# bd4sur/Nano

Hardware: AMD Instinct MI355X
Metric: decode_tokens_per_sec (higher is better)
Workload: dtype i8

## Files before the change

nano_amd/csrc/attn_impl.h:

```cpp
#pragma once
#include <hip/hip_fp16.h>
#include "device_common.h"
#include "kernels.h"

namespace nano {

namespace {

#ifndef NANO_GEMV_COMMON_H
#define DPP_F(v, ctrl) __int_as_float(__builtin_amdgcn_update_dpp(0, __float_as_int(v), (ctrl), 0xF, 0xF, true))
#endif

template <int W> __device__ __forceinline__ float group_sum_t(float v) {
    if (W >= 2) v += DPP_F(v, 0xB1);
    if (W >= 4) v += DPP_F(v, 0x4E);
    if (W >= 8) v += DPP_F(v, 0x141);
    if (W >= 16) v += DPP_F(v, 0x140);
    if (W >= 32) v += __shfl_xor(v, 16, 64);
    if (W >= 64) v += __shfl_xor(v, 32, 64);
    return v;
}
__device__ __forceinline__ float wave_sum_dpp(float v) {
    v += DPP_F(v, 0xB1); v += DPP_F(v, 0x4E); v += DPP_F(v, 0x141); v += DPP_F(v, 0x140);
    const float r0 = __int_as_float(__builtin_amdgcn_readlane(__float_as_int(v), 0));
// ... 46 lines not shown
    if constexpr (!KVH) row_base[elem] = v; else reinterpret_cast<__half *>(row_base)[elem] = __float2half_rn(v);
}
template <bool KVH> __device__ __forceinline__ KVRaw<KVH> kv_load4(__amdgpu_buffer_rsrc_t r, uint32_t off) {
    KVRaw<KVH> o;
    if constexpr (!KVH) o.v = bload_f4(r, off);
    else { typedef int i32x2 __attribute__((ext_vector_type(2))); const i32x2 t = __builtin_amdgcn_raw_buffer_load_b64(r, (int)off, 0, 0); o.v = make_uint2((uint32_t)t.x, (uint32_t)t.y); }
    return o;
}

typedef unsigned int u32x2_t __attribute__((ext_vector_type(2)));
__device__ __forceinline__ float xlane8(float v) { return __int_as_float(__builtin_amdgcn_update_dpp(0, __float_as_int(v), 0x128, 0xF, 0xF, true)); }
template <int LPR> __device__ __forceinline__ float xsub_sum(float v) {
    if (LPR <= 8) v += xlane8(v);
    { const u32x2_t r = __builtin_amdgcn_permlane16_swap(__float_as_uint(v), __float_as_uint(v), false, false); v = __uint_as_float(r[0]) + __uint_as_float(r[1]); }
    { const u32x2_t r = __builtin_amdgcn_permlane32_swap(__float_as_uint(v), __float_as_uint(v), false, false); v = __uint_as_float(r[0]) + __uint_as_float(r[1]); }
    return v;
}
template <int LPR> __device__ __forceinline__ float xsub_max(float v) {
    if (LPR <= 8) v = fmaxf(v, xlane8(v));
    { const u32x2_t r = __builtin_amdgcn_permlane16_swap(__float_as_uint(v), __float_as_uint(v), false, false); v = fmaxf(__uint_as_float(r[0]), __uint_as_float(r[1])); }
    { const u32x2_t r = __builtin_amdgcn_permlane32_swap(__float_as_uint(v), __float_as_uint(v), false, false); v = fmaxf(__uint_as_float(r[0]), __uint_as_float(r[1])); }
    return v;
}

__device__ __forceinline__ void combine_weights_lds(const float *mlh, uint32_t nsplit, float *wsh) {
    if (threadIdx.x < 64u) {
        const uint32_t s = threadIdx.x;
        const bool in = s < nsplit;
        const float mm = in ? mlh[2 * s] : -INFINITY;
        float v = in ? mlh[2 * s + 1] : 0.0f;
        float M = v > 0.0f ? mm : -INFINITY;
#pragma unroll
        for (int o = 32; o > 0; o >>= 1) M = fmaxf(M, __shfl_xor(M, o, 64));
        const float e = v > 0.0f ? expf(mm - M) : 0.0f;
        v = v * e;
        v += DPP_F(v, 0xB1); v += DPP_F(v, 0x4E); v += DPP_F(v, 0x141);
        float L = __int_as_float(__builtin_amdgcn_readlane(__float_as_int(v), 0));
        if (nsplit > 8u) {
            L += __int_as_float(__builtin_amdgcn_readlane(__float_as_int(v), 8));
            L += __int_as_float(__builtin_amdgcn_readlane(__float_as_int(v), 16));
            L += __int_as_float(__builtin_amdgcn_readlane(__float_as_int(v), 24));
        }
        if (nsplit > 32u) {
            L += __int_as_float(__builtin_amdgcn_readlane(__float_as_int(v), 32));
            L += __int_as_float(__builtin_amdgcn_readlane(__float_as_int(v), 40));
            L += __int_as_float(__builtin_amdgcn_readlane(__float_as_int(v), 48));
            L += __int_as_float(__builtin_amdgcn_readlane(__float_as_int(v), 56));
        }
        wsh[s] = e / L;
    }
    __syncthreads();
}
__device__ __forceinline__ uint32_t combine_slots(uint32_t nsplit) { return nsplit <= 8u ? 8u : nsplit <= 32u ? 32u : 64u; }

constexpr int NP = 2;

template <int LPR, int QV, int KVM, int MODE, bool KVH, bool PG, int NPT, bool W16, bool FUSE>
__device__ __forceinline__ void attention_body(const AttnArgs &a, unsigned char *smem, const uint32_t grp, const uint32_t b, const uint32_t split,
                                               const SlabHand &hh, const uint32_t hand_tag = 0u, const uint32_t hand_wait16 = 0u) {
    static_assert(!W16 || (KVH && QV % 4 == 0), "16-byte FP16 loads: two float4 slots per load");
    static_assert(!FUSE || (((MODE == 1 && LPR * QV * 4 == 128) || MODE == 2) && KVM == 1 && !KVH && !PG && LPR * QV * 4 <= 128),
                  "the fused launch: Qwen3 decode at head_dim 128, or the plain decode mode (no q/k norm, adjacent-pair RoPE: Nano) at head_dim <= 128; FP32 contiguous cache");
    constexpr int R = 256 / LPR;
    const int tid = threadIdx.x, lane = tid & 63;
    const int wid = __builtin_amdgcn_readfirstlane(tid >> 6);
    const uint32_t nsplit = a.nsplit;
    const uint32_t hd = (MODE == 1) ? (uint32_t)(QV * LPR * 4) : a.hd, half = hd >> 1, hd4 = (hd + 3) & ~3u;
    uint32_t kv_mul, g, h0;
    bool first_of_group;
    if constexpr (MODE != 0) {
        kv_mul = 1u << a.kvmul_log2;
        g = grp & ((1u << a.kv_log2) - 1u);
        const uint32_t sub_wg = grp >> a.kv_log2;
        h0 = (g << a.kvmul_log2) + sub_wg * KVM;
        first_of_group = sub_wg == 0;
    } else {
        kv_mul = a.n_head / a.n_kv_head;
        const bool xcd = a.kv_log2 != 0xffffffffu;
        g = xcd ? (grp & ((1u << a.kv_log2) - 1u)) : (grp * KVM) / kv_mul;
        h0 = xcd ? g * kv_mul + (grp >> a.kv_log2) * KVM : grp * KVM;
        first_of_group = (h0 % kv_mul) == 0;
    }
    constexpr bool G = MODE == 0;
    constexpr int VR = (KVM + 1 + 3) / 4;
    constexpr int JJ = (LPR == 16) ? 2 : 1;
    const bool fresh_k = G ? a.kraw != nullptr : true;
    const bool has_norm = G ? a.q_norm != nullptr : MODE == 1;
    const bool rq3 = G ? a.rope_qwen3 != 0 : MODE == 1;
    const bool has_rope = G ? a.rope_cos != nullptr : true;
    const uint32_t fixed_range = G ? a.fixed_range : 0u;
    const bool causal = G ? a.is_causal != 0 : true;
    float *const q_out = G ? a.q_out : nullptr;

    float *qh = reinterpret_cast<float *>(smem);
    float *kh = qh + KVM * hd4;
    float *redm = kh + hd4;
    float *redl = redm + KVM * 4;
    float *part = redl + KVM * 4;

    NANO_STAMP(a.stamps, 0, tid);
    if constexpr (MODE != 0)
        asm volatile("" :: "s"(a.q), "s"(a.kraw), "s"(a.kcache), "s"(a.vcache), "s"(a.pos), "s"(a.q_norm), "s"(a.k_norm), "s"(a.rope_cur),
                     "s"(a.out), "s"(a.ml), "s"(a.xba_out), "s"(a.nsplit), "s"(a.range_hint), "s"(a.layer), "s"(a.S), "s"(a.q_dim), "s"(a.kv_dim),
                     "s"(a.cache_bstride_rows), "s"(a.kv_log2), "s"(a.kvmul_log2), "s"(a.vraw), "s"(a.xf_out), "s"(a.pt_rows), "s"(a.kvrow));
    const uint32_t pos_ld = (MODE == 0 && a.fixed_range) ? 0u : a.pos[b];
    constexpr bool paged = PG;
    uint32_t prow_ld = 0u;
    if constexpr (PG) prow_ld = a.kvrow[b];
    constexpr uint32_t ESZ = KVH ? 2u : 4u;
    const size_t slot_rows = paged ? (size_t)a.layer * a.pool_rows : (size_t)b * a.cache_bstride_rows + (size_t)a.layer * a.S;
    const float *kc = reinterpret_cast<const float *>(reinterpret_cast<const unsigned char *>(a.kcache) + (slot_rows * a.kv_dim + (size_t)g * hd) * ESZ);
    const float *vc = reinterpret_cast<const float *>(reinterpret_cast<const unsigned char *>(a.vcache) + (slot_rows * a.kv_dim + (size_t)g * hd) * ESZ);
    const uint32_t cache_bytes = (paged ? a.pool_rows : fixed_range ? fixed_range : a.S) * a.kv_dim * ESZ;
    const __amdgpu_buffer_rsrc_t rk = mkrsrc(kc, cache_bytes - g * hd * ESZ);
    const __amdgpu_buffer_rsrc_t rv = mkrsrc(vc, cache_bytes - g * hd * ESZ);
    const uint32_t sub = (uint32_t)tid / LPR, j = (uint32_t)tid % LPR;
    auto fidx = [&](int q) -> uint32_t { return W16 ? 2u * (j + (uint32_t)LPR * (uint32_t)(q >> 1)) + (uint32_t)(q & 1) : j + (uint32_t)LPR * (uint32_t)q; };
    const uint32_t range_hint = fixed_range ? fixed_range : a.range_hint;

    constexpr bool REGQK = MODE != 0;
    constexpr bool SHARE = REGQK && !FUSE && KVM > 1;
    float4 qv[KVM][QV], kfresh[QV], vfresh[QV];
    float4 sv[SHARE ? QV : 1], snw[SHARE ? QV : 1];
    float4 qnw[QV], knw[QV], rcs[QV], rsn[QV];
    const __amdgpu_buffer_rsrc_t rq = mkrsrc(a.q + (size_t)b * a.q_dim, a.q_dim * 4u);
    const __amdgpu_buffer_rsrc_t rkr = mkrsrc(fresh_k ? a.kraw + (size_t)b * a.kv_dim : nullptr, fresh_k ? a.kv_dim * 4u : 0u);
    const bool fresh_v = KVH && a.vraw != nullptr;
    const __amdgpu_buffer_rsrc_t rvr = mkrsrc(fresh_v ? a.vraw + (size_t)b * a.kv_dim : nullptr, fresh_v ? a.kv_dim * 4u : 0u);
    const __amdgpu_buffer_rsrc_t rqn = mkrsrc(a.q_norm, has_norm ? hd * 4u : 0u);
    const __amdgpu_buffer_rsrc_t rkn = mkrsrc(a.k_norm, has_norm ? hd * 4u : 0u);
    float e0[VR][JJ], e1[VR][JJ], nw0[VR][JJ], nw1[VR][JJ];
    float rc[JJ], rs[JJ];
    const bool rope_staged = G ? (a.rope_cur != nullptr && fresh_k) : true;
    if constexpr (SHARE) {
        if (wid == 0) {
            const __amdgpu_buffer_rsrc_t rr = mkrsrc(a.rope_cur + (size_t)b * 2 * half, 2 * half * 4u);
            const bool isq = sub < (uint32_t)KVM, isk = sub == (uint32_t)KVM;
#pragma unroll
            for (int q = 0; q < QV; q++) {
                const uint32_t f = fidx(q);
                const uint32_t fo = (f * 4u < hd) ? f * 16u : OOB;
                const float4 xq = bload_f4(rq, (isq && fo != OOB) ? (h0 + sub) * hd * 4u + fo : OOB), xk = bload_f4(rkr, (isk && fo != OOB) ? g * hd * 4u + fo : OOB);
                sv[q] = isq ? xq : xk;
                if (MODE == 1) {
                    const float4 nq = bload_f4(rqn, isq ? fo : OOB), nk = bload_f4(rkn, isk ? fo : OOB);
                    snw[q] = isq ? nq : nk;
                    const uint32_t fr = f & (uint32_t)(QV * LPR / 2 - 1);
                    rcs[q] = bload_f4(rr, fo == OOB ? OOB : fr * 16u);
                    rsn[q] = bload_f4(rr, fo == OOB ? OOB : (half + fr * 4u) * 4u);
                } else {
                    const float c0 = bload_f(rr, fo == OOB ? OOB : (2u * f) * 4u), c1 = bload_f(rr, fo == OOB ? OOB : (2u * f + 1u) * 4u);
                    const float s0 = bload_f(rr, fo == OOB ? OOB : (half + 2u * f) * 4u), s1 = bload_f(rr, fo == OOB ? OOB : (half + 2u * f + 1u) * 4u);
                    rcs[q] = make_float4(c0, c1, 0.f, 0.f); rsn[q] = make_float4(s0, s1, 0.f, 0.f);
                }
            }
        }
        if constexpr (KVH) {
#pragma unroll
            for (int q = 0; q < QV; q++) { const uint32_t f = fidx(q); vfresh[q] = bload_f4(rvr, (f * 4u < hd) ? g * hd * 4u + f * 16u : OOB); }
        }
    } else if constexpr (REGQK) {
        const __amdgpu_buffer_rsrc_t rr = mkrsrc(a.rope_cur + (size_t)b * 2 * half, 2 * half * 4u);
#pragma unroll
        for (int q = 0; q < QV; q++) {
            const uint32_t f = fidx(q);
            const uint32_t fo = (f * 4u < hd) ? f * 16u : OOB;
// ... 28 lines not shown
            const uint32_t qb = (h0 + v) * hd * 4u, kb = g * hd * 4u;
            e0[vr][jj] = isq ? bload_f(rq, o0 + (ok ? qb : 0u)) : isk ? bload_f(rkr, o0 + (ok ? kb : 0u)) : 0.0f;
            e1[vr][jj] = isq ? bload_f(rq, o1 + (ok ? qb : 0u)) : isk ? bload_f(rkr, o1 + (ok ? kb : 0u)) : 0.0f;
            nw0[vr][jj] = !has_norm ? 1.0f : isq ? bload_f(rqn, o0) : isk ? bload_f(rkn, o0) : 0.0f;
            nw1[vr][jj] = !has_norm ? 1.0f : isq ? bload_f(rqn, o1) : isk ? bload_f(rkn, o1) : 0.0f;
        }
    }
    {
        const __amdgpu_buffer_rsrc_t rr = mkrsrc(rope_staged ? a.rope_cur + (size_t)b * 2 * half : nullptr, rope_staged ? 2 * half * 4u : 0u);
#pragma unroll
        for (int jj = 0; jj < JJ; jj++) {
            const uint32_t pi = (uint32_t)lane + 64u * jj;
            rc[jj] = bload_f(rr, pi < half ? pi * 4u : OOB);
            rs[jj] = bload_f(rr, pi < half ? (half + pi) * 4u : OOB);
        }
    }
    }
    KVRaw<KVH> kreg[NPT][QV], vreg[NPT][QV];
    auto issue_kv = [&](uint32_t round) {
#pragma unroll
        for (int p = 0; p < NPT; p++) {
            const uint32_t tb = ((round * NPT + p) * nsplit + split) * R, t = tb + sub;
            uint32_t row = t;
            if constexpr (PG) {
                const uint32_t blk = tb >> 6;
                uint32_t rb = 0xffffffffu;
                if (blk < a.pt_stride && tb < range_hint) {
                    const uint64_t pa = reinterpret_cast<uint64_t>(a.pt_rows + (size_t)b * a.pt_bstride + blk);
                    const uint64_t pu = ((uint64_t)(uint32_t)__builtin_amdgcn_readfirstlane((uint32_t)(pa >> 32)) << 32) | (uint64_t)(uint32_t)__builtin_amdgcn_readfirstlane((uint32_t)pa);
                    asm volatile("s_nop 4\n\ts_load_dword %0, %1, 0x0\n\ts_waitcnt lgkmcnt(0)" : "=s"(rb) : "s"(pu) : "memory");
                }
                row = rb == 0xffffffffu ? 0x7fffffu : rb + (t & 63u);
            }
#pragma unroll
            for (int q = 0; q < QV; q++) {
                const uint32_t f = fidx(q);
                const uint32_t off = (f * 4u < hd && t < range_hint && row < 0x7fffffu) ? (row * a.kv_dim + f * 4u) * ESZ : OOB;
                if constexpr (W16) {
                    if ((q & 1) == 0) {
                        const i32x4 kk = __builtin_amdgcn_raw_buffer_load_b128(rk, (int)off, 0, 0), vv = __builtin_amdgcn_raw_buffer_load_b128(rv, (int)off, 0, 0);
                        kreg[p][q].v = make_uint2((uint32_t)kk.x, (uint32_t)kk.y); kreg[p][q + 1].v = make_uint2((uint32_t)kk.z, (uint32_t)kk.w);
                        vreg[p][q].v = make_uint2((uint32_t)vv.x, (uint32_t)vv.y); vreg[p][q + 1].v = make_uint2((uint32_t)vv.z, (uint32_t)vv.w);
                    }
                } else {
                    kreg[p][q] = kv_load4<KVH>(rk, off);
                    vreg[p][q] = kv_load4<KVH>(rv, off);
                }
            }
        }
    };
    issue_kv(0);
    __builtin_amdgcn_sched_barrier(0);
    NANO_STAMP(a.stamps, 1, tid);
    if constexpr (FUSE) {
        float *vh = part + 4 * KVM * hd4;
        const uint32_t t7 = (uint32_t)tid & 127u;
        const unsigned long long *hand = hh.buf;
        const unsigned long long *g0p = (uint32_t)tid < 128u ? hand + (size_t)h0 * hd + t7 : hand + hh.base[1] + (size_t)g * hd + t7;
        const unsigned long long *g1p = hand + hh.base[2] + (size_t)g * hd + t7;
        const unsigned long long tag_done = (unsigned long long)hand_tag << 32;
        unsigned long long g0 = 0, g1 = 0;
        const bool live7 = MODE == 1 || t7 < hd;
        const bool two = (uint32_t)tid < 128u && live7;
        auto sweep = [&](unsigned long long &x0, unsigned long long &x1) {
            x0 = live7 ? __hip_atomic_load(g0p, __ATOMIC_RELAXED, __HIP_MEMORY_SCOPE_AGENT) : tag_done;
            x1 = two ? __hip_atomic_load(g1p, __ATOMIC_RELAXED, __HIP_MEMORY_SCOPE_AGENT) : tag_done;
        };
        auto ready = [&](unsigned long long x0, unsigned long long x1) { return __all((uint32_t)(x0 >> 32) == hand_tag && (uint32_t)(x1 >> 32) == hand_tag) != 0; };
        unsigned long long a0, a1, b0, b1;
        for (uint32_t w_ = 0; w_ < hand_wait16; w_++) __builtin_amdgcn_s_sleep(16);
        sweep(a0, a1);
        bool got = false;
        for (uint32_t spin = 0; spin < (1u << 13); spin++) {
            sweep(b0, b1);
            if (ready(a0, a1)) { g0 = a0; g1 = a1; got = true; break; }
            sweep(a0, a1);
            if (ready(b0, b1)) { g0 = b0; g1 = b1; got = true; break; }
            if ((spin & 63u) == 63u && hand_aborted(hh)) break;
        }
        if (live7) {
            if ((uint32_t)tid < 128u) { qh[t7] = __uint_as_float((uint32_t)g0); vh[t7] = __uint_as_float((uint32_t)g1); }
            else kh[t7] = __uint_as_float((uint32_t)g0);
        }
        if (__syncthreads_or(got ? 0 : 1)) {
            if (!got && lane == 0) hand_give_up(hh, a.err);
            return;
        }
#pragma unroll
        for (int q = 0; q < QV; q++) {
            const uint32_t f = fidx(q);
            const bool in = MODE == 1 || f * 4u < hd;
            const float4 z4 = make_float4(0.f, 0.f, 0.f, 0.f);
            qv[0][q] = in ? *reinterpret_cast<const float4 *>(qh + 4u * f) : z4;
            kfresh[q] = in ? *reinterpret_cast<const float4 *>(kh + 4u * f) : z4;
            vfresh[q] = in ? *reinterpret_cast<const float4 *>(vh + 4u * f) : z4;
        }
    }

    const uint32_t pos = fixed_range ? (fixed_range - 1) : pos_ld;
    const uint32_t prow = paged ? prow_ld : pos;
    const uint32_t range = fixed_range ? fixed_range : (causal ? (pos + 1) : a.S);
    if constexpr (SHARE) {
        if (wid == 0) {
            const bool isq = sub < (uint32_t)KVM, isk = sub == (uint32_t)KVM;
            if (MODE == 1) {
                float ssq = 0.0f;
#pragma unroll
                for (int q = 0; q < QV; q++) { ssq += sv[q].x * sv[q].x; ssq += sv[q].y * sv[q].y; ssq += sv[q].z * sv[q].z; ssq += sv[q].w * sv[q].w; }
                ssq = group_sum_t<LPR>(ssq); ssq /= (float)hd; ssq += 1e-5f; ssq = 1.0f / sqrtf(ssq);
#pragma unroll
                for (int q = 0; q < QV; q++) {
                    sv[q].x = snw[q].x * (ssq * sv[q].x); sv[q].y = snw[q].y * (ssq * sv[q].y); sv[q].z = snw[q].z * (ssq * sv[q].z); sv[q].w = snw[q].w * (ssq * sv[q].w);
                }
#pragma unroll
                for (int q = 0; q < QV / 2; q++) {
                    const float4 l = sv[q], h = sv[q + QV / 2], c = rcs[q], sn = rsn[q];
                    sv[q].x = l.x * c.x - h.x * sn.x; sv[q + QV / 2].x = h.x * c.x + l.x * sn.x;
                    sv[q].y = l.y * c.y - h.y * sn.y; sv[q + QV / 2].y = h.y * c.y + l.y * sn.y;
                    sv[q].z = l.z * c.z - h.z * sn.z; sv[q + QV / 2].z = h.z * c.z + l.z * sn.z;
                    sv[q].w = l.w * c.w - h.w * sn.w; sv[q + QV / 2].w = h.w * c.w + l.w * sn.w;
                }
            } else {
#pragma unroll
                for (int q = 0; q < QV; q++) {
                    const float4 t = sv[q], c = rcs[q], sn = rsn[q];
                    sv[q].x = t.x * c.x - t.y * sn.x; sv[q].y = t.x * sn.x + t.y * c.x;
                    sv[q].z = t.z * c.y - t.w * sn.y; sv[q].w = t.z * sn.y + t.w * c.y;
                }
            }
            if (isk) {
#pragma unroll
                for (int q = 0; q < QV; q++) sv[q] = kv_round<KVH>(sv[q]);
            }
            if (isq || isk) {
                float *dst = isq ? qh + sub * hd4 : kh;
#pragma unroll
                for (int q = 0; q < QV; q++) { const uint32_t f = fidx(q); if (f * 4u < hd) *reinterpret_cast<float4 *>(dst + 4u * f) = sv[q]; }
            }
            if (isk && split == 0 && first_of_group) {
                float *krow = reinterpret_cast<float *>(reinterpret_cast<unsigned char *>(const_cast<float *>(kc)) + (size_t)prow * a.kv_dim * ESZ);
                float *vrow = reinterpret_cast<float *>(reinterpret_cast<unsigned char *>(const_cast<float *>(vc)) + (size_t)prow * a.kv_dim * ESZ);
#pragma unroll
                for (int q = 0; q < QV; q++) {
                    const uint32_t f = fidx(q);
                    if (f * 4u < hd) { kv_store4<KVH>(krow, 4u * f, sv[q]); if (KVH && fresh_v) kv_store4<KVH>(vrow, 4u * f, kv_round<KVH>(vfresh[q])); }
                }
            }
        }
        if (a.prep_only) return;
        __syncthreads();
#pragma unroll
        for (int q = 0; q < QV; q++) {
            const uint32_t f = fidx(q);
            const bool ok = f * 4u < hd;
#pragma unroll
            for (int m = 0; m < KVM; m++) qv[m][q] = ok ? *reinterpret_cast<const float4 *>(qh + m * hd4 + 4 * f) : make_float4(0.f, 0.f, 0.f, 0.f);
            kfresh[q] = ok ? *reinterpret_cast<const float4 *>(kh + 4 * f) : make_float4(0.f, 0.f, 0.f, 0.f);
            if (KVH) vfresh[q] = kv_round<KVH>(vfresh[q]);
        }
    } else if constexpr (REGQK) {
        if (MODE == 1) {
            float sk = 0.0f, sq[KVM];
#pragma unroll
            for (int m = 0; m < KVM; m++) sq[m] = 0.0f;
#pragma unroll
            for (int q = 0; q < QV; q++) {
                sk += kfresh[q].x * kfresh[q].x; sk += kfresh[q].y * kfresh[q].y; sk += kfresh[q].z * kfresh[q].z; sk += kfresh[q].w * kfresh[q].w;
// ... 57 lines not shown
            const uint32_t pi = (uint32_t)lane + 64u * jj;
            const bool ok = has_rope && pi < half && fresh_k;
            rc[jj] = ok ? a.rope_cos[(size_t)pos * half + pi] : 1.0f;
            rs[jj] = ok ? a.rope_sin[(size_t)pos * half + pi] : 0.0f;
        }
    }
#pragma unroll
    for (int vr = 0; vr < VR; vr++) {
        const uint32_t v = (uint32_t)wid + 4u * vr;
        if (v <= (uint32_t)KVM) {
            const bool isk = v == (uint32_t)KVM;
            float x0[JJ], x1[JJ];
#pragma unroll
            for (int jj = 0; jj < JJ; jj++) { x0[jj] = e0[vr][jj]; x1[jj] = e1[vr][jj]; }
            if (fresh_k && has_norm) {
                float acc = 0.0f;
#pragma unroll
                for (int jj = 0; jj < JJ; jj++) { acc += x0[jj] * x0[jj]; acc += x1[jj] * x1[jj]; }
                float ss = wave_sum_dpp(acc);
                ss /= (float)hd; ss += 1e-5f; ss = 1.0f / sqrtf(ss);
#pragma unroll
                for (int jj = 0; jj < JJ; jj++) { x0[jj] = nw0[vr][jj] * (ss * x0[jj]); x1[jj] = nw1[vr][jj] * (ss * x1[jj]); }
            }
            float *dst = isk ? kh : qh + v * hd4;
#pragma unroll
            for (int jj = 0; jj < JJ; jj++) {
                const uint32_t pi = (uint32_t)lane + 64u * jj;
                if (pi < half && (!isk || fresh_k)) {
                    const uint32_t i0 = rq3 ? pi : 2 * pi, i1 = rq3 ? pi + half : 2 * pi + 1;
                    float y0 = x0[jj], y1 = x1[jj];
                    if (fresh_k && has_rope) {
                        const float c = rc[jj], s = rs[jj];
                        if (rq3) { y0 = x0[jj] * c - x1[jj] * s; y1 = x1[jj] * c + x0[jj] * s; }
                        else { y0 = x0[jj] * c - x1[jj] * s; y1 = x0[jj] * s + x1[jj] * c; }
                    }
                    if (isk) { y0 = kv_round1<KVH>(y0); y1 = kv_round1<KVH>(y1); }
                    dst[i0] = y0; dst[i1] = y1;
                    if (isk && split == 0 && first_of_group) {
                        float *krow = reinterpret_cast<float *>(reinterpret_cast<unsigned char *>(const_cast<float *>(kc)) + (size_t)prow * a.kv_dim * ESZ);
                        kv_store1<KVH>(krow, i0, y0); kv_store1<KVH>(krow, i1, y1);
                    }
                    if (!isk && split == 0 && q_out) { float *qo = q_out + (size_t)b * a.q_dim + (size_t)(h0 + v) * hd; qo[i0] = y0; qo[i1] = y1; }
                }
            }
        }
    }
    if constexpr (KVH) {
#pragma unroll
        for (int q = 0; q < QV; q++) {
            const uint32_t f = fidx(q);
            const bool ok = f * 4u < hd;
            vfresh[q] = kv_round<KVH>(bload_f4(rvr, ok ? g * hd * 4u + f * 16u : OOB));
            if (fresh_v && ok && split == 0 && sub == 0 && first_of_group)
                kv_store4<KVH>(reinterpret_cast<float *>(reinterpret_cast<unsigned char *>(const_cast<float *>(vc)) + (size_t)prow * a.kv_dim * ESZ), 4u * f, vfresh[q]);
        }
    }
    __syncthreads();
    if (a.prep_only) return;

#pragma unroll
    for (int q = 0; q < QV; q++) {
        const uint32_t f = fidx(q);
        const bool ok = f * 4u < hd;
#pragma unroll
        for (int m = 0; m < KVM; m++) qv[m][q] = ok ? *reinterpret_cast<const float4 *>(qh + m * hd4 + 4 * f) : make_float4(0.f, 0.f, 0.f, 0.f);
        kfresh[q] = (ok && fresh_k) ? *reinterpret_cast<const float4 *>(kh + 4 * f) : make_float4(0.f, 0.f, 0.f, 0.f);
    }
    }
    NANO_STAMP(a.stamps, 2, qv[0][0].x);
    const float sq_hd = sqrtf((float)hd);
    float mrun[KVM], lrun[KVM];
    float4 acc[KVM][QV];
#pragma unroll
    for (int m = 0; m < KVM; m++) {
        mrun[m] = -INFINITY; lrun[m] = 0.0f;
#pragma unroll
        for (int q = 0; q < QV; q++) acc[m][q] = make_float4(0.f, 0.f, 0.f, 0.f);
    }
    const uint32_t per_round = NPT * nsplit * R;
    const uint32_t limit = range < range_hint ? range : range_hint;
    const uint32_t nround = (limit + per_round - 1) / per_round;
    for (uint32_t round = 0; round < nround; round++) {
        if (round) issue_kv(round);
        float sc[KVM][NPT];
#pragma unroll
        for (int p = 0; p < NPT; p++) {
            const uint32_t t = ((round * NPT + p) * nsplit + split) * R + sub;
            const bool fresh = fresh_k && t == pos;
#pragma unroll
            for (int m = 0; m < KVM; m++) {
                float d = 0.0f;
#pragma unroll
                for (int q = 0; q < QV; q++) {
                    const float4 kk = fresh ? kfresh[q] : kv_cvt(kreg[p][q]);
                    d = __builtin_fmaf(qv[m][q].x, kk.x, d); d = __builtin_fmaf(qv[m][q].y, kk.y, d); d = __builtin_fmaf(qv[m][q].z, kk.z, d); d = __builtin_fmaf(qv[m][q].w, kk.w, d);
                }
                d = group_sum_t<LPR>(d);
                sc[m][p] = (t < range) ? d / sq_hd : -INFINITY;
            }
        }
#pragma unroll
        for (int m = 0; m < KVM; m++) {
            float mx = mrun[m];
#pragma unroll
            for (int p = 0; p < NPT; p++) mx = fmaxf(mx, sc[m][p]);
            const float scale = (mrun[m] == -INFINITY) ? 0.0f : expf(mrun[m] - mx);
            float l = lrun[m] * scale;
#pragma unroll
            for (int q = 0; q < QV; q++) { acc[m][q].x *= scale; acc[m][q].y *= scale; acc[m][q].z *= scale; acc[m][q].w *= scale; }
#pragma unroll
            for (int p = 0; p < NPT; p++) {
                const float e = (sc[m][p] == -INFINITY) ? 0.0f : expf(sc[m][p] - mx);
                l += e;
                const uint32_t tv = ((round * NPT + p) * nsplit + split) * R + sub;
                const bool vf = (FUSE || (KVH && fresh_v)) && tv == pos;
#pragma unroll
                for (int q = 0; q < QV; q++) {
                    const float4 vv = vf ? vfresh[q] : kv_cvt(vreg[p][q]);
                    acc[m][q].x = __builtin_fmaf(e, vv.x, acc[m][q].x); acc[m][q].y = __builtin_fmaf(e, vv.y, acc[m][q].y);
                    acc[m][q].z = __builtin_fmaf(e, vv.z, acc[m][q].z); acc[m][q].w = __builtin_fmaf(e, vv.w, acc[m][q].w);
                }
            }
            mrun[m] = mx; lrun[m] = l;
        }
    }

    NANO_STAMP(a.stamps, 3, acc[0][0].x);
    if constexpr (KVM > 1) {
        constexpr int NS = 64 / LPR, HP = LPR * QV * 4;
        float *tr = part + 4 * KVM * hd4 + (size_t)wid * NS * HP;
        const uint32_t sw = (uint32_t)lane / LPR;
#pragma unroll
        for (int m = 0; m < KVM; m++) {
            const float Mw = xsub_max<LPR>(mrun[m]);
            const float w = (mrun[m] == -INFINITY) ? 0.0f : expf(mrun[m] - Mw);
            const float lw = xsub_sum<LPR>(lrun[m] * w);
#pragma unroll
            for (int q = 0; q < QV; q++)
                *reinterpret_cast<float4 *>(tr + sw * HP + 4u * fidx(q)) = make_float4(acc[m][q].x * w, acc[m][q].y * w, acc[m][q].z * w, acc[m][q].w * w);
            for (uint32_t o = (uint32_t)lane * 2u; o < (uint32_t)HP; o += 128u) {
                float2 v[NS];
#pragma unroll
                for (int k = 0; k < NS; k++) v[k] = *reinterpret_cast<const float2 *>(tr + k * HP + o);
                float2 t;
                if constexpr (NS == 8) {
                    t.x = ((v[0].x + v[1].x) + (v[2].x + v[3].x)) + ((v[4].x + v[5].x) + (v[6].x + v[7].x));
                    t.y = ((v[0].y + v[1].y) + (v[2].y + v[3].y)) + ((v[4].y + v[5].y) + (v[6].y + v[7].y));
                } else {
                    t.x = (v[0].x + v[1].x) + (v[2].x + v[3].x);
                    t.y = (v[0].y + v[1].y) + (v[2].y + v[3].y);
                }
                if (o < hd) *reinterpret_cast<float2 *>(part + ((size_t)wid * KVM + m) * hd4 + o) = t;
            }
            if (lane == 0) { redm[m * 4 + wid] = Mw; redl[m * 4 + wid] = lw; }
        }
    } else {
#pragma unroll
    for (int m = 0; m < KVM; m++) {
        const float Mw = xsub_max<LPR>(mrun[m]);
        const float w = (mrun[m] == -INFINITY) ? 0.0f : expf(mrun[m] - Mw);
        const float lw = xsub_sum<LPR>(lrun[m] * w);
#pragma unroll
        for (int q = 0; q < QV; q++) {
            const float4 t = make_float4(xsub_sum<LPR>(acc[m][q].x * w), xsub_sum<LPR>(acc[m][q].y * w), xsub_sum<LPR>(acc[m][q].z * w), xsub_sum<LPR>(acc[m][q].w * w));
            const uint32_t f = fidx(q);
            if (lane < LPR && f * 4u < hd) *reinterpret_cast<float4 *>(part + ((size_t)wid * KVM + m) * hd4 + 4 * f) = t;
        }
        if (lane == 0) { redm[m * 4 + wid] = Mw; redl[m * 4 + wid] = lw; }
    }
    }
    __syncthreads();
    NANO_STAMP(a.stamps, 4, redl[0]);
    for (uint32_t idx = tid; idx < (uint32_t)KVM * hd; idx += 256) {
        uint32_t m = 0, i = idx;
        if (KVM > 1) { m = idx / hd; i = idx - m * hd; }
        const float4 mw = *reinterpret_cast<const float4 *>(redm + m * 4), lw4 = *reinterpret_cast<const float4 *>(redl + m * 4);
        const float M = fmaxf(fmaxf(mw.x, mw.y), fmaxf(mw.z, mw.w));
        const float e0 = (mw.x == -INFINITY) ? 0.0f : expf(mw.x - M), e1 = (mw.y == -INFINITY) ? 0.0f : expf(mw.y - M);
        const float e2 = (mw.z == -INFINITY) ? 0.0f : expf(mw.z - M), e3 = (mw.w == -INFINITY) ? 0.0f : expf(mw.w - M);
        const float *pp = part + (size_t)m * hd4 + i;
        const size_t ws_ = (size_t)KVM * hd4;
        float L = lw4.x * e0; L += lw4.y * e1; L += lw4.z * e2; L += lw4.w * e3;
        float o = pp[0] * e0; o += pp[ws_] * e1; o += pp[2 * ws_] * e2; o += pp[3 * ws_] * e3;
        const uint32_t h = h0 + m;
        if (nsplit == 1) {
            const float val = o / L;
            a.xba_out[(size_t)b * a.q_dim + (size_t)h * hd + i] = val;
            if (a.xf_out) {
                float mx = fabsf(val);
#pragma unroll
                for (int o2 = 1; o2 < 64; o2 <<= 1) mx = fmaxf(mx, __shfl_xor(mx, o2, 64));
                const float scale = div_const<127>(mx);
                const uint32_t e = h * hd + i, g = e >> 6, jj = e & 63u, ng = a.q_dim >> 6;
                const size_t gb = (size_t)(b >> 4) * ng + g;
                a.xf_out[gb * 1024u + (size_t)((jj >> 4) * 16u + (b & 15u)) * 16u + (jj & 15u)] = (int8_t)q80_quant1(val, scale);
                if (jj == 0) a.xsf_out[gb * 16u + (b & 15u)] = scale;
            }
        } else {
            a.out[((size_t)b * nsplit + split) * a.q_dim + (size_t)h * hd + i] = o;
            if (i == 0) { float *ml = a.ml + (((size_t)b * a.n_head + h) * nsplit + split) * 2; ml[0] = M; ml[1] = L; }
        }
    }
    NANO_STAMP_END(a.stamps, 5);
}

template <int LPR, int QV, int KVM, int MODE, bool KVH, bool PG, int NPT, bool W16>
__global__ __launch_bounds__(256) void attention_kernel(const AttnArgs a) {
    extern __shared__ __attribute__((aligned(16))) unsigned char smem[];
    attention_body<LPR, QV, KVM, MODE, KVH, PG, NPT, W16, false>(a, smem, blockIdx.x, blockIdx.y, blockIdx.z, SlabHand{});
}


}
// ... 3 lines not shown
```

nano_amd/csrc/gemv_q4k_chunk.hip:

```cpp
#include "gemv_q4k_impl.h"
#include <hip/hip_ext.h>

namespace nano {

extern hipEvent_t g_q80_probe_start, g_q80_probe_stop;

namespace {

template <int ROLE, int NV, int D, bool LOOP, int NB = 1>
__global__ __launch_bounds__(1024) void gemv_q4k_chunk_kernel(const GemvDev a) {
    static_assert(NB == 1 || (ROLE == R_GENERIC && NV == 1), "several sequences: activations arrive quantized (q4k_quant_rows_kernel), generic role");
    extern __shared__ __attribute__((aligned(16))) unsigned char smem[];
#define CHUNK_A a
#define CHUNK_BID blockIdx.x
#define CHUNK_HAND 0
#define CHUNK_HANDV (SlabHand{})
#define CHUNK_PTAG 0u
#include "gemv_q4k_chunk_body.inc"
#undef CHUNK_A
#undef CHUNK_BID
#undef CHUNK_HAND
#undef CHUNK_HANDV
#undef CHUNK_PTAG
}
// ... 150 lines not shown
template <int ROLE, int NV>
hipError_t launch_quant_rows_t(const GemvDev &d, XGroup *out, uint32_t nb, size_t lds, hipStream_t st) {
    auto kern = &q4k_quant_rows_kernel<ROLE, NV>;
    if (lds > 64 * 1024) (void)hipFuncSetAttribute(reinterpret_cast<const void *>(kern), hipFuncAttributeMaxDynamicSharedMemorySize, (int)lds);
    hipLaunchKernelGGL(kern, dim3(nb), dim3(d.nthr), lds, st, d, out);
    return hipGetLastError();
}
template <int NV>
hipError_t launch_quant_rows_r(const GemvDev &d, XGroup *out, uint32_t nb, size_t lds, hipStream_t st) {
    if (d.flags == F_NORM) return launch_quant_rows_t<R_NORM_STORE, NV>(d, out, nb, lds, st);
    if (d.flags == 0) return launch_quant_rows_t<R_RESID, NV>(d, out, nb, lds, st);
    if (d.flags == F_COMBINE) return launch_quant_rows_t<R_RESID_COMBINE, NV>(d, out, nb, lds, st);
    return launch_quant_rows_t<R_GENERIC, NV>(d, out, nb, lds, st);
}

}

bool gemv_q4k_chunk_supports(const GemvArgs &a) {
    ChunkPlan p;
    if (a.nb <= 1) return plan_chunk(a, p);
    GemvArgs one = a; one.nb = 1;
    return a.q4_scratch && (size_t)a.nb * (a.n >> 5) * sizeof(XGroup) <= a.q4_scratch_bytes && plan_chunk(one, p) && plan_chunk(a, p);
}
bool gemv_q4k_chunk_loops(const GemvArgs &a) { ChunkPlan p; return a.nb == 1 && plan_chunk(a, p) && p.loop; }
uint32_t gemv_q4k_chunk_partials(const GemvArgs &a) {
    ChunkPlan p;
    if (a.nb != 1 || !a.tile_max || a.epi != GEMV_EPI_STORE || a.nseg != 1 || a.seg[0].out_pstride || !plan_chunk(a, p)) return 0;
    return p.grid;
}

static hipError_t launch_gemv_q4k_chunk_batched(GemvArgs &a, hipStream_t st) {
    if (!gemv_q4k_chunk_supports(a)) return hipErrorInvalidValue;
    ChunkPlan p1, p;
    GemvArgs one = a; one.nb = 1;
    if (!plan_chunk(one, p1) || !plan_chunk(a, p)) return hipErrorInvalidValue;
    const uint32_t bpl = a.n >> 8, GT = bpl * 8u;
    XGroup *xg = reinterpret_cast<XGroup *>(a.q4_scratch);
    {
        GemvDev q = to_dev(a);
        q.nthr = p1.nthr; q.tile_max = nullptr;
        const size_t lds = (size_t)GT * sizeof(XGroup) + (16 + (a.attn_part ? (size_t)a.attn_n_head * 8 : 0)) * 4 + 16;
        const hipError_t e = p1.nv <= 1 ? launch_quant_rows_r<1>(q, xg, a.nb, lds, st) : p1.nv <= 2 ? launch_quant_rows_r<2>(q, xg, a.nb, lds, st) : launch_quant_rows_r<4>(q, xg, a.nb, lds, st);
        if (e != hipSuccess) return e;
    }
    GemvArgs g = a;
    g.norm_w = nullptr; g.attn_part = nullptr; g.attn_ml = nullptr; g.tile_max = nullptr;
    GemvDev d = to_dev(g);
    d.flags = F_PRE; d.xq_in = reinterpret_cast<const int8_t *>(xg);
    d.rw = p.rw; d.nthr = p.nthr; d.units = p.rounds;
    d.magic_nchunk = (uint32_t)(((1ull << 32) + bpl - 1) / bpl);
    const uint32_t nseg = a.epi == GEMV_EPI_SWIGLU ? 1u : a.nseg;
    d.wg_c0 = nseg > 1 ? p.wg[0] : 0xffffffffu;
    d.wg_c1 = nseg > 2 ? p.wg[0] + p.wg[1] : 0xffffffffu;
    d.ntiles = 0;
    if (a.nb <= 2) return launch_chunk_nb<2>(d, p, st);
    if (a.nb <= 4) return launch_chunk_nb<4>(d, p, st);
    return launch_chunk_nb<8>(d, p, st);
}

static bool q4k_fused_shape(const GemvArgs &ga, const AttnArgs &aa, ChunkPlan &p) {
    if (ga.nb != 1 || ga.nseg != 3 || ga.epi != GEMV_EPI_STORE || !ga.norm_w || ga.xq_in || ga.x4_in || ga.attn_part || ga.tile_max || ga.resid_add) return false;
    if (ga.seg[0].out_pstride || ga.seg[1].out_pstride) return false;
    if (ga.n > 1024u || !plan_chunk(ga, p, 4u) || p.loop || p.nthr != 256u || p.nv != 1u) return false;
    if (p.lds > 64u * 1024u) return false;
    return fused_attn_side_ok(aa, ga.seg[0].rows, ga.seg[1].rows, ga.seg[2].rows);
}
bool qkv_attn_fused_q4k_supports(const GemvArgs &ga, const AttnArgs &aa) { ChunkPlan p; return q4k_fused_shape(ga, aa, p); }

hipError_t launch_qkv_attn_fused_q4k(const GemvArgs &ga, const AttnArgs &aa, unsigned long long *hand, uint32_t *tick, uint32_t layer1, hipStream_t st) {
    ChunkPlan p;
    if (!hand || !tick || !layer1 || layer1 > 127u || !q4k_fused_shape(ga, aa, p)) return hipErrorInvalidValue;
    GemvDev d = to_dev(ga);
    d.tile_max = nullptr; d.ntiles = 0;
    const uint32_t bpl = ga.n >> 8;
    d.rw = p.rw; d.nthr = p.nthr; d.units = p.rounds;
    d.magic_nchunk = (uint32_t)(((1ull << 32) + bpl - 1) / bpl);
    d.wg_c0 = p.wg[0]; d.wg_c1 = p.wg[0] + p.wg[1];
    AttnArgs a = aa;
    { uint32_t l2 = 0; while ((1u << l2) < a.n_kv_head) l2++; a.kv_log2 = l2; }
    { const uint32_t kv_mul = a.n_head / a.n_kv_head; uint32_t l2 = 0; while ((1u << l2) < kv_mul) l2++; a.kvmul_log2 = l2; }
    SlabHand h{};
    h.buf = hand; h.tick = tick; h.layer1 = layer1;
    h.base[0] = 0; h.base[1] = a.q_dim; h.base[2] = a.q_dim + a.kv_dim;
    const size_t hd4 = a.hd, lds_a = (hd4 + hd4 + 4 + 4 + 4 * hd4 + hd4) * sizeof(float);
    const size_t lds = p.lds > lds_a ? p.lds : lds_a;
    Q4FusedArgs fa{};
    fa.g = d; fa.a = a; fa.hand = h; fa.n_attn = a.n_head * a.nsplit; fa.head_wgs = a.n_head; fa.ngemv = p.grid;
    fa.wait16 = 0u;
#define Q4F_GO(NV_, D_) do { hipLaunchKernelGGL((q4k_qkv_attn_fused_kernel<NV_, D_>), dim3(fa.n_attn + fa.ngemv), dim3(p.nthr), lds, st, fa); return hipGetLastError(); } while (0)
#define Q4F_NV(NV_) do { if (p.d == 1) Q4F_GO(NV_, 1); if (p.d == 2) Q4F_GO(NV_, 2); if (p.d == 4) Q4F_GO(NV_, 4); Q4F_GO(NV_, 8); } while (0)
    if (p.nv <= 1) Q4F_NV(1);
    if (p.nv <= 2) Q4F_NV(2);
    Q4F_NV(4);
#undef Q4F_NV
#undef Q4F_GO
}

hipError_t launch_gemv_q4k_chunk(GemvArgs &a, hipStream_t st) {
    if (a.nb > 1) return launch_gemv_q4k_chunk_batched(a, st);
    ChunkPlan p;
    if (!plan_chunk(a, p)) return hipErrorInvalidValue;
    GemvDev d = to_dev(a);
    if (a.x4_in) { d.flags |= F_PRE; d.xq_in = reinterpret_cast<const int8_t *>(a.x4_in); }
    const uint32_t bpl = a.n >> 8;
    d.rw = p.rw; d.nthr = p.nthr; d.units = p.rounds;
    d.magic_nchunk = (uint32_t)(((1ull << 32) + bpl - 1) / bpl);
    const uint32_t nseg = a.epi == GEMV_EPI_SWIGLU ? 1u : a.nseg;
    d.wg_c0 = nseg > 1 ? p.wg[0] : 0xffffffffu;
    d.wg_c1 = nseg > 2 ? p.wg[0] + p.wg[1] : 0xffffffffu;
    d.ntiles = gemv_q4k_chunk_partials(a);
    if (!d.ntiles) d.tile_max = nullptr;
    const uint32_t f = d.flags;
    if (f == F_NORM && d.epi == GEMV_EPI_STORE) return launch_chunk_r<R_NORM_STORE>(d, p, st);
    if (f == 0 && d.epi == GEMV_EPI_RESID) return launch_chunk_r<R_RESID>(d, p, st);
    if (f == F_COMBINE && d.epi == GEMV_EPI_RESID) return launch_chunk_r<R_RESID_COMBINE>(d, p, st);
    if (f == F_NORM && d.epi == GEMV_EPI_SWIGLU) return launch_chunk_r<R_NORM_SWIGLU>(d, p, st);
    return launch_chunk_r<R_GENERIC>(d, p, st);
}

}
```

nano_amd/csrc/gemv_q80_impl.h:

```cpp
#include <string.h>
#include <stdio.h>
#include "gemv_common.h"
#include "gemv_q80_host.h"

namespace nano {

namespace {


__device__ __forceinline__ void quant_store4(float4 v, float scale, int8_t *dst) {
    const int q0 = q80_quant1(v.x, scale), q1 = q80_quant1(v.y, scale), q2 = q80_quant1(v.z, scale), q3 = q80_quant1(v.w, scale);
    *reinterpret_cast<uint32_t *>(dst) = (uint32_t)(q0 & 0xff) | ((uint32_t)(q1 & 0xff) << 8) | ((uint32_t)(q2 & 0xff) << 16) | ((uint32_t)(q3 & 0xff) << 24);
}

template <int ROLE, int GS, int B, int NV>
__device__ __forceinline__ void stage_finish(const GemvDev &a, Staged<B, NV> &r, int8_t *xq, float *xs, float *red, uint32_t n16, uint32_t ng4) {
    const uint32_t tid = threadIdx.x, nthr = a.nthr, n = a.n, ng = a.ng;
    const uint32_t lane = tid & 63u, wid = tid >> 6, NW = nthr >> 6;
    if (has_flag<ROLE>(a, F_PRE)) {
        for (uint32_t b = 0; b < a.nb; b++) {
            for (uint32_t i = tid * 16u; i < n; i += nthr * 16u) *reinterpret_cast<int4 *>(xq + b * n16 + i) = *reinterpret_cast<const int4 *>(a.xq_in + (size_t)b * n16 + i);
            for (uint32_t i = tid; i < ng; i += nthr) xs[b * ng4 + i] = a.xs_in[(size_t)b * ng + i];
        }
        __syncthreads();
// ... 612 lines not shown

struct Wo13Plan { SlabPlan a, b; uint32_t nw, nv_a, upw_a, wa, wb; int sig; };
static bool wo13_shape(const GemvArgs &wo, const GemvArgs &w13, Wo13Plan &q) {
    if (wo.gs != 64 || w13.gs != 64 || wo.nb != 1 || w13.nb != 1 || !q80_canonical(wo) || !q80_canonical(w13)) return false;
    if (wo.nseg != 1 || wo.epi != GEMV_EPI_RESID || wo.norm_w || wo.xq_in || wo.tile_max || wo.resid_add || wo.seg[0].out_pstride) return false;
    if (wo.attn_part && (wo.attn_nsplit > 8u || wo.attn_hd % 4u)) return false;
    if (w13.nseg != 2 || w13.epi != GEMV_EPI_SWIGLU || !w13.norm_w || w13.xq_in || w13.attn_part || w13.tile_max || w13.resid_add) return false;
    if (use_stream(wo) || use_stream(w13) || w13.n != wo.seg[0].rows || w13.xin != wo.seg[0].out || w13.n % 4u) return false;
    q.a = plan_slab(wo, 1); q.b = plan_slab(w13, 1);
    q.nw = q.b.nw;
    const uint32_t units_a = ((q.a.rw + 3) / 4) * ((wo.n + 1023) / 1024);
    q.upw_a = (units_a + q.nw - 1) / q.nw;
    q.nv_a = (wo.n / 4 + 64 * q.nw - 1) / (64 * q.nw);
    q.wa = (wo.seg[0].rows + q.a.rw - 1) / q.a.rw; q.wb = (w13.seg[0].rows + q.b.rw - 1) / q.b.rw;
    const uint32_t cus = w13.cus ? w13.cus : 256u;
    if (q.wa > q.wb || q.wb > cus) return false;
    if (q.a.rw > 64 * q.nw || q.b.rw > 64 * q.nw) return false;
    q.sig = 0;
    if (q.nw == 4u && q.nv_a == 2u && q.upw_a == 1u && q.b.nv == 1u && q.b.upw == 2u) q.sig = 1;
    if (q.sig == 1) {
        const uint32_t units_b = ((q.b.rw + 3) / 4) * ((w13.n + 1023) / 1024) * 2u;
        if ((units_a + 7u) / 8u == 1u && (wo.n / 4 + 511u) / 512u == 1u && (units_b + 7u) / 8u == 1u && (w13.n / 4 + 511u) / 512u == 1u) { q.sig = 3; q.nw = 8u; }
    }
    return q.sig != 0;
}
static void slab_dev_fill(GemvDev &d, const GemvArgs &a, const SlabPlan &p, uint32_t nthr) {
    d.tile_max = nullptr;
    d.rw = p.rw; d.tpw = (p.rw + 3) / 4; d.magic_rw = 65536u / p.rw + 1u; d.log2_tiles = 0;
    d.units = d.tpw * d.nchunk * (a.epi == GEMV_EPI_SWIGLU ? 2u : 1u);
    d.wg_c0 = 0xffffffffu; d.wg_c1 = 0xffffffffu;
    d.nthr = nthr;
}
static size_t slab_lds(const GemvDev &d) {
    const uint32_t nmat = d.epi == GEMV_EPI_SWIGLU ? 2 : 1;
    const size_t n16 = (d.n + 15) & ~15u, ng4 = (d.ng + 3) & ~3u, pitch = ((d.ng + 47) / 64) * 64 + 16;
    return n16 + ng4 * 4 + 64 + ((d.flags & F_COMBINE) ? (size_t)d.attn_n_head * 32 : 0) + (size_t)nmat * (d.tpw * 4) * pitch * 4;
}

#endif

template <int GS, int B>
static hipError_t launch_b(const GemvArgs &a, hipStream_t st) {
    GemvDev d = to_dev(a);
    if (use_stream(a)) return launch_stream_b<GS, B>(d, st);
    d.tile_max = nullptr;
    return launch_slab_b<GS, B>(d, a, st);
}
template <int GS>
static hipError_t launch_gs(const GemvArgs &a, hipStream_t st) {
    if (a.nb <= 1) return launch_b<GS, 1>(a, st);
    if (a.nb <= 2) return launch_b<GS, 2>(a, st);
    if (a.nb <= 4) return launch_b<GS, 4>(a, st);
    return launch_b<GS, 8>(a, st);
}

}

hipError_t NANO_Q80_ENTRY(const GemvArgs &a, hipStream_t st) { return launch_gs<NANO_Q80_GS>(a, st); }

#if NANO_Q80_GS == 64
bool qkv_attn_fused_supports(const GemvArgs &ga, const AttnArgs &aa) { SlabPlan p; return fused_shape(ga, aa, p); }

hipError_t launch_qkv_attn_fused(const GemvArgs &ga, const AttnArgs &aa, unsigned long long *hand, uint32_t *tick, uint32_t layer1, hipStream_t st) {
    SlabPlan p;
    if (!hand || !tick || !layer1 || layer1 > 127u || !fused_shape(ga, aa, p)) return hipErrorInvalidValue;
    GemvDev d = to_dev(ga);
    d.tile_max = nullptr;
    d.rw = p.rw; d.tpw = (p.rw + 3) / 4; d.magic_rw = 65536u / p.rw + 1u; d.log2_tiles = 0;
    d.units = d.tpw * d.nchunk;
    uint32_t wg[3];
    for (uint32_t s2 = 0; s2 < 3; s2++) wg[s2] = (ga.seg[s2].rows + p.rw - 1) / p.rw;
    d.wg_c0 = wg[0]; d.wg_c1 = wg[0] + wg[1];
    const uint32_t ngemv = wg[0] + wg[1] + wg[2];
    d.nthr = 256;
    AttnArgs a = aa;
    { uint32_t l2 = 0; while ((1u << l2) < a.n_kv_head) l2++; a.kv_log2 = l2; }
    { const uint32_t kv_mul = a.n_head / a.n_kv_head; uint32_t l2 = 0; while ((1u << l2) < kv_mul) l2++; a.kvmul_log2 = l2; }
    SlabHand h{};
    h.buf = hand; h.tick = tick; h.layer1 = layer1;
    h.base[0] = 0; h.base[1] = a.q_dim; h.base[2] = a.q_dim + a.kv_dim;
    const uint32_t n_attn = a.n_head * a.nsplit;
    const size_t n16 = (d.n + 15) & ~15u, ng4 = (d.ng + 3) & ~3u, pitch = ((d.ng + 47) / 64) * 64 + 16;
    const size_t lds_g = n16 + ng4 * 4 + 64 + (size_t)(d.tpw * 4) * pitch * 4;
    const size_t hd4 = a.hd, lds_a = (hd4 + hd4 + 4 + 4 + 4 * hd4 + hd4) * sizeof(float);
    const size_t lds = lds_g > lds_a ? lds_g : lds_a;
    if (lds > 64 * 1024) return hipErrorInvalidValue;
    const int upw = p.upw <= 1 ? 1 : p.upw <= 2 ? 2 : 4;
    FusedArgs fa{};
    fa.g = d; fa.a = a; fa.hand = h; fa.n_attn = n_attn; fa.head_wgs = a.n_head; fa.ngemv = ngemv;
    fa.wait16 = 1u;
#define FUSED_GO(NV_, UPW_) do { hipLaunchKernelGGL((qkv_attn_fused_kernel<NV_, UPW_>), dim3(n_attn + ngemv), dim3(256), lds, st, fa); return hipGetLastError(); } while (0)
#define FUSED_NV(NV_) do { if (upw == 1) FUSED_GO(NV_, 1); if (upw == 2) FUSED_GO(NV_, 2); FUSED_GO(NV_, 4); } while (0)
    if (p.nv == 1u) FUSED_NV(1);
    if (p.nv == 2u) FUSED_NV(2);
    FUSED_NV(4);
#undef FUSED_NV
#undef FUSED_GO
}

bool wo_w13_fused_supports(const GemvArgs &wo, const GemvArgs &w13) { Wo13Plan q; return wo13_shape(wo, w13, q); }

hipError_t launch_wo_w13_fused(const GemvArgs &wo, const GemvArgs &w13, unsigned long long *hand, uint32_t *tick, uint32_t layer1, hipStream_t st) {
    Wo13Plan q;
    if (!hand || !tick || !layer1 || layer1 > 127u || !wo13_shape(wo, w13, q)) return hipErrorInvalidValue;
    Wo13Args fa{};
    fa.wo = to_dev(wo); fa.w13 = to_dev(w13);
    slab_dev_fill(fa.wo, wo, q.a, 64 * q.nw); slab_dev_fill(fa.w13, w13, q.b, 64 * q.nw);
    fa.wo_wgs = q.wa;
    fa.wait16 = 4u;
    SlabHand h{};
    h.buf = hand; h.tick = tick; h.layer1 = layer1;
    h.base[0] = 0; h.base[1] = 0; h.base[2] = 0;
    fa.hand = h;
    const size_t la = slab_lds(fa.wo), lb = slab_lds(fa.w13), lds = la > lb ? la : lb;
    if (lds > 64 * 1024) return hipErrorInvalidValue;
    const bool comb = (fa.wo.flags & F_COMBINE) != 0;
#define WO13_GO(RA_, NVA_, UA_, NVB_, UB_, NT_) do { hipLaunchKernelGGL((wo_w13_fused_kernel<RA_, NVA_, UA_, NVB_, UB_, NT_>), dim3(q.wb), dim3(NT_), lds, st, fa); return hipGetLastError(); } while (0)
    if (q.sig == 1) { if (comb) WO13_GO(R_RESID_COMBINE, 2, 1, 1, 2, 256); WO13_GO(R_RESID, 2, 1, 1, 2, 256); }
    if (comb) WO13_GO(R_RESID_COMBINE, 1, 1, 1, 1, 512);
    WO13_GO(R_RESID, 1, 1, 1, 1, 512);
#undef WO13_GO
}
#endif

}
```

Baseline: 1928.

## Add specialized fast path for fused single-head attention decode

For one specific fused attention configuration, the fresh K/V values are patched into the register buffers once per round. This replaces the per-element select between fresh and cached values inside the dot-product and accumulate loops. The block-wide syncthreads_or is swapped for an LDS flag array read as a uint4, and the cross-lane transpose reduction used for KVM>1 is also enabled for this path. LDS sizing grows to hold the extra flag and transpose scratch space, which may lower occupancy or hit the 64KB limit for larger head dims.

```diff
diff --git a/nano_amd/csrc/attn_impl.h b/nano_amd/csrc/attn_impl.h
--- a/nano_amd/csrc/attn_impl.h
+++ b/nano_amd/csrc/attn_impl.h
@@ -152,6 +152,7 @@
         first_of_group = (h0 % kv_mul) == 0;
     }
     constexpr bool G = MODE == 0;
+    constexpr bool FAST = FUSE && MODE == 1 && KVM == 1 && LPR == 8 && QV == 4 && NPT == 2 && !KVH && !PG && !W16;
     constexpr int VR = (KVM + 1 + 3) / 4;
     constexpr int JJ = (LPR == 16) ? 2 : 1;
     const bool fresh_k = G ? a.kraw != nullptr : true;
@@ -346,7 +347,16 @@
             if ((uint32_t)tid < 128u) { qh[t7] = __uint_as_float((uint32_t)g0); vh[t7] = __uint_as_float((uint32_t)g1); }
             else kh[t7] = __uint_as_float((uint32_t)g0);
         }
-        if (__syncthreads_or(got ? 0 : 1)) {
+        if constexpr (FAST) {
+            uint32_t *gave = reinterpret_cast<uint32_t *>(vh + hd4);
+            if (lane == 0) gave[wid] = got ? 0u : 1u;
+            __syncthreads();
+            const uint4 gv = *reinterpret_cast<const uint4 *>(gave);
+            if (gv.x | gv.y | gv.z | gv.w) {
+                if (!got && lane == 0) hand_give_up(hh, a.err);
+                return;
+            }
+        } else if (__syncthreads_or(got ? 0 : 1)) {
             if (!got && lane == 0) hand_give_up(hh, a.err);
             return;
         }
@@ -570,11 +580,21 @@
     const uint32_t nround = (limit + per_round - 1) / per_round;
     for (uint32_t round = 0; round < nround; round++) {
         if (round) issue_kv(round);
+        if constexpr (FAST) {
+#pragma unroll
+            for (int p = 0; p < NPT; p++) {
+                const uint32_t t = ((round * NPT + p) * nsplit + split) * R + sub;
+                if (__any(t == pos) && t == pos) {
+#pragma unroll
+                    for (int q = 0; q < QV; q++) { kreg[p][q].v = kfresh[q]; vreg[p][q].v = vfresh[q]; }
+                }
+            }
+        }
         float sc[KVM][NPT];
 #pragma unroll
         for (int p = 0; p < NPT; p++) {
             const uint32_t t = ((round * NPT + p) * nsplit + split) * R + sub;
-            const bool fresh = fresh_k && t == pos;
+            const bool fresh = !FAST && fresh_k && t == pos;
 #pragma unroll
             for (int m = 0; m < KVM; m++) {
                 float d = 0.0f;
@@ -601,7 +621,7 @@
                 const float e = (sc[m][p] == -INFINITY) ? 0.0f : expf(sc[m][p] - mx);
                 l += e;
                 const uint32_t tv = ((round * NPT + p) * nsplit + split) * R + sub;
-                const bool vf = (FUSE || (KVH && fresh_v)) && tv == pos;
+                const bool vf = !FAST && (FUSE || (KVH && fresh_v)) && tv == pos;
 #pragma unroll
                 for (int q = 0; q < QV; q++) {
                     const float4 vv = vf ? vfresh[q] : kv_cvt(vreg[p][q]);
@@ -614,9 +634,9 @@
     }
 
     NANO_STAMP(a.stamps, 3, acc[0][0].x);
-    if constexpr (KVM > 1) {
+    if constexpr (KVM > 1 || FAST) {
         constexpr int NS = 64 / LPR, HP = LPR * QV * 4;
-        float *tr = part + 4 * KVM * hd4 + (size_t)wid * NS * HP;
+        float *tr = part + 4 * KVM * hd4 + (FAST ? hd4 + 4 : 0) + (size_t)wid * NS * HP;
         const uint32_t sw = (uint32_t)lane / LPR;
 #pragma unroll
         for (int m = 0; m < KVM; m++) {
diff --git a/nano_amd/csrc/gemv_q4k_chunk.hip b/nano_amd/csrc/gemv_q4k_chunk.hip
--- a/nano_amd/csrc/gemv_q4k_chunk.hip
+++ b/nano_amd/csrc/gemv_q4k_chunk.hip
@@ -256,7 +256,7 @@
     SlabHand h{};
     h.buf = hand; h.tick = tick; h.layer1 = layer1;
     h.base[0] = 0; h.base[1] = a.q_dim; h.base[2] = a.q_dim + a.kv_dim;
-    const size_t hd4 = a.hd, lds_a = (hd4 + hd4 + 4 + 4 + 4 * hd4 + hd4) * sizeof(float);
+    const size_t hd4 = a.hd, lds_a = (hd4 + hd4 + 4 + 4 + 4 * hd4 + hd4 + 4 + 4 * 8 * hd4) * sizeof(float);
     const size_t lds = p.lds > lds_a ? p.lds : lds_a;
     Q4FusedArgs fa{};
     fa.g = d; fa.a = a; fa.hand = h; fa.n_attn = a.n_head * a.nsplit; fa.head_wgs = a.n_head; fa.ngemv = p.grid;
diff --git a/nano_amd/csrc/gemv_q80_impl.h b/nano_amd/csrc/gemv_q80_impl.h
--- a/nano_amd/csrc/gemv_q80_impl.h
+++ b/nano_amd/csrc/gemv_q80_impl.h
@@ -718,7 +718,7 @@
     const uint32_t n_attn = a.n_head * a.nsplit;
     const size_t n16 = (d.n + 15) & ~15u, ng4 = (d.ng + 3) & ~3u, pitch = ((d.ng + 47) / 64) * 64 + 16;
     const size_t lds_g = n16 + ng4 * 4 + 64 + (size_t)(d.tpw * 4) * pitch * 4;
-    const size_t hd4 = a.hd, lds_a = (hd4 + hd4 + 4 + 4 + 4 * hd4 + hd4) * sizeof(float);
+    const size_t hd4 = a.hd, lds_a = (hd4 + hd4 + 4 + 4 + 4 * hd4 + hd4 + 4 + 4 * 8 * hd4) * sizeof(float);
     const size_t lds = lds_g > lds_a ? lds_g : lds_a;
     if (lds > 64 * 1024) return hipErrorInvalidValue;
     const int upw = p.upw <= 1 ? 1 : p.upw <= 2 ? 2 : 4;
```

New measurement: 1966 (median of 6 runs). 2.0% higher.
